# FFmpeg/FFmpeg

Hardware: AMD Instinct MI355X
Metric: swscale_nv12_1080p_to_4k_bicubic_Mpixels_per_s (higher is better)
Workload: dtype u8

## Files before the change

### ffmpeg_amd/csrc/kernels/sws_kernels.h

```cpp
#ifndef FFHIP_SWS_KERNELS_H
#define FFHIP_SWS_KERNELS_H

#include <hip/hip_runtime.h>
#include <stddef.h>
#include <stdint.h>

__host__ __device__ __forceinline__ uint32_t sws_block_numbering(uint32_t b, uint32_t nb, int mode)
{
    if (mode == 1) {
        const uint32_t x = b & 7u, sl = b >> 3, q = nb >> 3, r = nb & 7u;
        return (x < r ? x * (q + 1u) : r * (q + 1u) + (x - r) * q) + sl;
    }
    if (mode > 1) {
        const uint32_t lg = (uint32_t)mode - 1u, C = 1u << lg, full = nb & ~(8u * C - 1u);
        if (b < full) {
            const uint32_t x = b & 7u, sl = b >> 3;
            return (((sl >> lg) << 3) + x) * C + (sl & (C - 1u));
        }
    }
    return b;
}

struct FFHipYuv2RgbK {
    int cy;
// ... 27 lines not shown

struct FFHipDevFilter {
    const int16_t *filter;
    const int32_t *pos;
    int size, n;
};

struct FFHipScalePlaneArgs {
    const uint8_t *src[2];
    uint8_t *dst[2];
    ptrdiff_t src_stride[2], dst_stride[2];
    size_t src_fp[2], dst_fp[2];
    int src_step, dst_step;
    int srcW, srcH, dstW, dstH;
    int nframes;
    FFHipDevFilter h, v;
    int tw, th;
    int max_cols, max_rows;
    int tiles_x, tiles_y;
    int rc_coeff, rc_offset, rc_clip;
};
int ffhip_launch_scale_yuv(const FFHipScalePlaneArgs &lum, const FFHipScalePlaneArgs &chr, hipStream_t stream);
int ffhip_plan_scale_plane(FFHipScalePlaneArgs *a, int channels, const int32_t *hpos_host, const int32_t *vpos_host);


struct FFHipCwJob {
    const uint8_t *src[2];
    uint8_t *dst[2];
    ptrdiff_t sstride[2], dstride[2];
    size_t sfp[2], dfp[2];
    int kind, src_swap, dst_swap;
    int srcW, srcH, dstW, dstH;
    const int16_t *hf; const int32_t *hp;
    const int16_t *vf; const int32_t *vp;
    int ncb, nstrips, strip_rows, unit_begin;
};
struct FFHipCwArgs {
    FFHipCwJob job[3];
    int njobs, units_per_frame, nframes, flags;
};
int  ffhip_cw_bank_nowrap(const int16_t *filter, int size, int n);
int  ffhip_cw_bank_dup12(const int32_t *hpos, int hn);
int  ffhip_cw_bank_ok(const int32_t *hpos, int hsize, int hn, int srcW, const int32_t *vpos, int vsize, int vn, int srcH);
void ffhip_cw_plan_job(FFHipCwJob *j, int groups_per_lane, int strip_target);
int  ffhip_launch_colwalk(FFHipCwArgs &A, int luma_groups, int depth, hipStream_t stream);

struct FFHipUp2Job {
    const uint8_t *src; uint8_t *dst;
    ptrdiff_t sstride, dstride;
    size_t sfp, dfp;
    int pair, swap;
    int srcW, srcH;
    int ngroups;
    const uint32_t *hfv;
    const uint32_t *vfv;
    int nfull, upj;
    int nstrips, steps_per_strip, unit_begin;
    int hb_sdepth, hb_ddepth, hb_smsb, hb_dmsb;
    int rc_coeff, rc_offset;
    uint32_t hco[16];
    int hco_ok;
};
struct FFHipUp2Args {
    FFHipUp2Job job[3];
    int njobs, units_per_pack, npacks, nframes, fshift;
    int xcd;
};
#ifdef __cplusplus
#include <vector>
int  ffhip_up2_virtual_bank(const int16_t *filter, const int32_t *pos, int n_dst, int n_src, std::vector<uint32_t> *out);
int  ffhip_up2_hco(const std::vector<uint32_t> &h, uint32_t out[16]);
#endif
void ffhip_up2_plan_job(FFHipUp2Job *j, int lanes_per_frame, int want_steps);
int  ffhip_launch_up2(FFHipUp2Args &A, int depth, int var, hipStream_t stream);

struct FFHipUp2RgbArgs {
    const uint8_t *src[3];
    uint8_t *dst;
    ptrdiff_t sstride[3], dstride;
    size_t sfp[3], dfp;
    int sil, swap;
    int srcW, srcH;
    int ngroups;
    int nframes;
    const uint32_t *hco;
    const uint32_t *vt;
    int nstrips, steps_per_strip;
    int fpp, wpp, npacks;
    int vround;
    int lay;
    FFHipYuv2RgbK k;
};
#ifdef __cplusplus
int  ffhip_upn_virtual_bank(const int16_t *filter, const int32_t *pos, int n_dst, int n_src, int ratio, std::vector<uint32_t> *out);
int  ffhip_up2rgb_hco(const std::vector<uint32_t> &hl, const std::vector<uint32_t> &hc, uint32_t out[32]);
#endif
void ffhip_up2rgb_plan(FFHipUp2RgbArgs *a, int want_steps, int fpp_forced);
int  ffhip_launch_up2rgb(FFHipUp2RgbArgs &A, int var, hipStream_t stream);

struct FFHipDn2Job {
    const uint8_t *src; uint8_t *dst;
    ptrdiff_t sstride, dstride;
    size_t sfp, dfp;
    int pair, swap;
    int srcH, dstH;
    int ngroups;
// ... 303 lines not shown
```

### ffmpeg_amd/csrc/kernels/sws_up2.hip

```cpp
#include <stdlib.h>
#include <type_traits>
#include <vector>

#include "common.h"
#include "sws_kernels.h"

typedef uint32_t up_u2 __attribute__((ext_vector_type(2)));
typedef uint32_t up_u3 __attribute__((ext_vector_type(3)));
typedef uint32_t up_u4 __attribute__((ext_vector_type(4)));
typedef uint32_t up_u8 __attribute__((ext_vector_type(8)));
typedef up_u3 __attribute__((aligned(4))) up_u3a;
typedef const uint8_t __attribute__((address_space(1))) *up_gcp;
typedef uint8_t __attribute__((address_space(1))) *up_gp;
typedef const up_u3a __attribute__((address_space(1))) *up_gc3;
typedef up_u2 __attribute__((address_space(1))) *up_g2;
typedef up_u4 __attribute__((aligned(4))) up_u4a;
typedef up_u2 __attribute__((aligned(4))) up_u2a;
typedef const up_u4a __attribute__((address_space(1))) *up_gc4;
typedef const up_u2a __attribute__((address_space(1))) *up_gc2;
typedef up_u4a __attribute__((address_space(1))) *up_g4;
typedef const up_u8 __attribute__((address_space(4))) *up_cc8;

struct UpRaw { uint32_t q[3]; };
struct UpRawH { uint32_t q[6]; };
// ... 96 lines not shown

__device__ __forceinline__ void up_v8h(uint32_t (&w)[4], const uint32_t (&pa)[8], const uint32_t (&pb)[8], uint32_t f01, uint32_t f23,
                                       int kround, int sh, uint32_t maxpk)
{
    int t0, t1, t2, t3, t4, t5, t6, t7;
    asm("v_dot2_i32_i16 %4, %12, %28, %30\n\t"
        "v_dot2_i32_i16 %5, %13, %28, %30\n\t"
        "v_dot2_i32_i16 %6, %14, %28, %30\n\t"
        "v_dot2_i32_i16 %7, %15, %28, %30\n\t"
        "v_dot2_i32_i16 %8, %16, %28, %30\n\t"
        "v_dot2_i32_i16 %9, %17, %28, %30\n\t"
        "v_dot2_i32_i16 %10, %18, %28, %30\n\t"
        "v_dot2_i32_i16 %11, %19, %28, %30\n\t"
        "v_dot2_i32_i16 %4, %20, %29, %4\n\t"
        "v_dot2_i32_i16 %5, %21, %29, %5\n\t"
        "v_dot2_i32_i16 %6, %22, %29, %6\n\t"
        "v_dot2_i32_i16 %7, %23, %29, %7\n\t"
        "v_dot2_i32_i16 %8, %24, %29, %8\n\t"
        "v_dot2_i32_i16 %9, %25, %29, %9\n\t"
        "v_dot2_i32_i16 %10, %26, %29, %10\n\t"
        "v_dot2_i32_i16 %11, %27, %29, %11\n\t"
        "v_ashrrev_i32 %4, %31, %4\n\t"
        "v_ashrrev_i32 %5, %31, %5\n\t"
        "v_ashrrev_i32 %6, %31, %6\n\t"
        "v_ashrrev_i32 %7, %31, %7\n\t"
        "v_ashrrev_i32 %8, %31, %8\n\t"
        "v_ashrrev_i32 %9, %31, %9\n\t"
        "v_ashrrev_i32 %10, %31, %10\n\t"
        "v_ashrrev_i32 %11, %31, %11\n\t"
        "v_cvt_pk_i16_i32 %0, %4, %5\n\t"
        "v_cvt_pk_i16_i32 %1, %6, %7\n\t"
        "v_cvt_pk_i16_i32 %2, %8, %9\n\t"
        "v_cvt_pk_i16_i32 %3, %10, %11\n\t"
        "v_pk_max_i16 %0, %0, 0\n\t"
        "v_pk_max_i16 %1, %1, 0\n\t"
        "v_pk_max_i16 %2, %2, 0\n\t"
        "v_pk_max_i16 %3, %3, 0\n\t"
        "v_pk_min_i16 %0, %0, %32\n\t"
        "v_pk_min_i16 %1, %1, %32\n\t"
        "v_pk_min_i16 %2, %2, %32\n\t"
        "v_pk_min_i16 %3, %3, %32"
        : "=&v"(w[0]), "=&v"(w[1]), "=&v"(w[2]), "=&v"(w[3]), "=&v"(t0), "=&v"(t1), "=&v"(t2), "=&v"(t3), "=&v"(t4), "=&v"(t5), "=&v"(t6),
          "=&v"(t7)
        : "v"(pa[0]), "v"(pa[1]), "v"(pa[2]), "v"(pa[3]), "v"(pa[4]), "v"(pa[5]), "v"(pa[6]), "v"(pa[7]),
          "v"(pb[0]), "v"(pb[1]), "v"(pb[2]), "v"(pb[3]), "v"(pb[4]), "v"(pb[5]), "v"(pb[6]), "v"(pb[7]),
          "s"(f01), "s"(f23), "v"(kround), "v"(sh), "v"(maxpk));
}

template <int PAIR, int D, int VAR, int HB = 0, int RC = 0, int SC = 0>
__device__ __forceinline__ void up2_unit(const FFHipUp2Job &J, int frame0, int fshift, int gbase, int strip, int lane, int nframes)
{
    constexpr bool DBG_NOST = VAR & 16, DBG_ROW0 = VAR & 32, DBG_COPY = VAR & 64;
    constexpr bool NTS = VAR & 1;
    const int lpf = 64 >> fshift;
    const int fsub = lane >> (6 - fshift);
    const int gl = lane & (lpf - 1);
    const int graw = gbase + gl, fraw = frame0 + fsub;
    const bool act = graw < J.ngroups && fraw < nframes;
    const int g = min(graw, J.ngroups - 1);
    const int fs = fraw < nframes ? fsub : 0;
    const bool lb = g == 0, rb = g == J.ngroups - 1;
    const bool border = gbase == 0 || gbase + lpf >= J.ngroups;

    const uint32_t soff = (uint32_t)fs * (uint32_t)J.sfp +
                          (uint32_t)(!HB ? (lb ? 0 : rb ? 4 * g - 8 : 4 * g - 4)
                                     : PAIR ? (lb ? 0 : rb ? 8 * g - 16 : 8 * g - 8) : (lb ? 0 : rb ? 8 * g - 8 : 8 * g - 4));
    const uint32_t doff = (uint32_t)fs * (uint32_t)J.dfp + (HB ? 16u : 8u) * (uint32_t)g;
    const int hsh = HB ? J.hb_sdepth - 1 : 7, vsh = HB ? 27 - J.hb_ddepth : 19;
    const uint32_t maxpk = HB ? ((1u << J.hb_ddepth) - 1) * 0x00010001u : 0;
    const int smsb = HB ? (J.hb_smsb ? 16 - J.hb_sdepth : 0) : 0, dmsb = HB ? (J.hb_dmsb ? 16 - J.hb_ddepth : 0) : 0;

    constexpr int NCF = SC ? 4 : PAIR ? 8 : 16;
    uint32_t cf[NCF];
    if (!SC) {
        const up_u4 *p = reinterpret_cast<const up_u4 *>(J.hfv) + (size_t)g * (NCF / 4);
#pragma unroll
        for (int i = 0; i < NCF / 4; i++) {
            const up_u4 v = p[i];
            cf[4 * i] = v.x; cf[4 * i + 1] = v.y; cf[4 * i + 2] = v.z; cf[4 * i + 3] = v.w;
        }
    }
    const uint32_t cE0 = J.hco[0], cE1 = J.hco[1], cO0 = J.hco[2], cO1 = J.hco[3];
    const uint32_t par = PAIR ? (J.swap ? 0x00010001u : 0u) : 0u;
    const uint32_t sA0 = 0x0c020c00u + par, sA1 = 0x0c040c02u + par, sA2 = 0x0c060c04u + par;
    const uint32_t sB0 = 0x0c030c01u - par, sB1 = 0x0c050c03u - par, sB2 = 0x0c070c05u - par;
    const uint32_t fixl = PAIR ? 0x01000100u : 0x00000000u, fixr = PAIR ? 0x03020302u : 0x03030303u;

    const int S = J.steps_per_strip;
    const int a = 1 + strip * S, b = min(a + S, J.srcH + 2);
    const uint8_t *sbase = J.src + (size_t)frame0 * J.sfp;
    uint8_t *dbase = J.dst + (size_t)frame0 * J.dfp;
    const ptrdiff_t sstride = J.sstride, dstride = J.dstride;
    const int srcH = J.srcH, dstH = 2 * J.srcH;
    int pr = a - 3;
    const uint8_t *pf = sbase + (ptrdiff_t)min(max(pr, 0), srcH - 1) * sstride;
    uint8_t *dr = dbase + (ptrdiff_t)(2 * a - 3) * dstride;
    asm("" : "+s"(pf), "+s"(dr));

    typedef typename std::conditional<HB != 0, UpRawH, UpRaw>::type Raw;
    auto load_next = [&](Raw &o) {
        uint32_t off = soff;
        asm volatile("" : "+v"(off));
        if (HB) {
            const up_u4 w = *(up_gc4)((up_gcp)pf + off);
            o.q[0] = w.x; o.q[1] = w.y; o.q[2] = w.z; o.q[3] = w.w;
            if (PAIR) {
                const up_u2 x = *(up_gc2)((up_gcp)pf + off + 16);
                o.q[4] = x.x; o.q[5] = x.y;
            }
        } else {
            const up_u3 w = *(up_gc3)((up_gcp)pf + off);
            o.q[0] = w.x; o.q[1] = w.y; o.q[2] = w.z;
        }
        pr++;
        if (!DBG_ROW0)
            pf += (pr >= 1 && pr <= srcH - 1) ? sstride : 0;
        asm("" : "+s"(pf));
    };

    uint32_t ring[3][8];
    int hprev[8];
#pragma unroll
    for (int i = 0; i < 8; i++)
        hprev[i] = 0;
    int kround = HB ? 1 << (vsh - 1) : 64 << 12;
    asm volatile("" : "+v"(kround));

    auto hpass = [&](const Raw &w, uint32_t (&Pnew)[8]) {
        int h[8];
        if (HB) {
            uint32_t v[6];
            constexpr int NQ = PAIR ? 6 : 4;
#pragma unroll
            for (int i = 0; i < NQ; i++)
                v[i] = w.q[i];
            if (border) {
                if (PAIR) {
                    const uint32_t q0 = w.q[0], q1 = w.q[1], q2 = w.q[2], q3 = w.q[3], q4 = w.q[4], q5 = w.q[5];
                    v[0] = lb ? q0 : rb ? q2 : q0; v[1] = lb ? q0 : rb ? q3 : q1; v[2] = lb ? q0 : rb ? q4 : q2;
                    v[3] = lb ? q1 : rb ? q5 : q3; v[4] = lb ? q2 : rb ? q5 : q4; v[5] = lb ? q3 : rb ? q5 : q5;
                } else {
                    const uint32_t q0 = w.q[0], q1 = w.q[1], q2 = w.q[2], q3 = w.q[3];
                    const uint32_t f0 = __builtin_amdgcn_perm(q0, q0, 0x01000100u), f3 = __builtin_amdgcn_perm(q3, q3, 0x03020302u);
                    v[0] = lb ? f0 : rb ? q1 : q0; v[1] = lb ? q0 : rb ? q2 : q1;
                    v[2] = lb ? q1 : rb ? q3 : q2; v[3] = lb ? q2 : rb ? f3 : q3;
                }
            }
            if (smsb) {
                typedef unsigned short up_h2 __attribute__((ext_vector_type(2)));
#pragma unroll
                for (int i = 0; i < NQ; i++)
                    v[i] = __builtin_bit_cast(uint32_t, __builtin_bit_cast(up_h2, v[i]) >> (unsigned short)smsb);
            }
            if (PAIR) {
                uint32_t a[5], b[5];
#pragma unroll
                for (int k = 0; k < 5; k++) {
                    a[k] = __builtin_amdgcn_perm(v[k + 1], v[k], 0x05040100u);
                    b[k] = __builtin_amdgcn_perm(v[k + 1], v[k], 0x07060302u);
                }
                int ha[4], hb[4];
                up_h4s(ha, a[0], a[1], a[1], a[2], a[2], a[3], a[3], a[4], cf, hsh);
                up_h4s(hb, b[0], b[1], b[1], b[2], b[2], b[3], b[3], b[4], cf, hsh);
#pragma unroll
                for (int i = 0; i < 4; i++) {
                    h[2 * i] = ha[i];
                    h[2 * i + 1] = hb[i];
                }
            } else {
                const uint32_t p0 = v[0], p2 = v[1], p4 = v[2], p6 = v[3];
                const uint32_t p1 = __builtin_amdgcn_alignbyte(v[1], v[0], 2), p3 = __builtin_amdgcn_alignbyte(v[2], v[1], 2);
                const uint32_t p5 = __builtin_amdgcn_alignbyte(v[3], v[2], 2);
                int hl[4], hh[4];
                up_h4s(hl, p0, p1, p1, p2, p2, p3, p3, p4, cf, hsh);
                up_h4s(hh, p2, p3, p3, p4, p4, p5, p5, p6, cf + 8, hsh);
#pragma unroll
                for (int i = 0; i < 4; i++) {
                    h[i] = hl[i];
                    h[4 + i] = hh[i];
                }
            }
#pragma unroll
            for (int i = 0; i < 8; i++) {
// ... 232 lines not shown
    return 1;
}

int ffhip_up2_hco(const std::vector<uint32_t> &v, uint32_t out[16])
{
    const int n = (int)(v.size() / 2);
    if (n < 16 || (n & 1))
        return 0;
    for (int x = 3; x < n - 3; x++)
        if (v[2 * (size_t)x] != v[2 * (size_t)(4 + (x & 1))] || v[2 * (size_t)x + 1] != v[2 * (size_t)(4 + (x & 1)) + 1])
            return 0;
    for (int i = 0; i < 4; i++)
        out[i] = v[8 + i];
    for (int i = 0; i < 6; i++) {
        out[4 + i] = v[i];
        out[10 + i] = v[2 * (size_t)(n - 3) + i];
    }
    return 1;
}

void ffhip_up2_plan_job(FFHipUp2Job *j, int lanes_per_frame, int want)
{
    const int steps = j->srcH + 1;
    int n = cdiv(steps, want);
    int s = cdiv(cdiv(steps, n), 6) * 6;
    j->steps_per_strip = s;
    j->nstrips = cdiv(steps, s);
    if (lanes_per_frame == 64) {
        j->nfull = 0;
        j->upj = cdiv(j->ngroups, 64);
    } else {
        j->nfull = j->ngroups / 64;
        j->upj = j->nfull * (64 / lanes_per_frame) + cdiv(j->ngroups - j->nfull * 64, lanes_per_frame);
    }
}

int ffhip_launch_up2(FFHipUp2Args &A, int depth, int var, hipStream_t stream)
{
    if (A.nframes <= 0)
        return 0;
    int u = 0;
    for (int i = 0; i < A.njobs; i++) {
        A.job[i].unit_begin = u;
        u += A.job[i].upj * A.job[i].nstrips;
    }
    A.units_per_pack = u;
    A.npacks = (A.nframes + (1 << A.fshift) - 1) >> A.fshift;
    const long long waves = (long long)u * A.npacks;
    if (waves >= (1LL << 31)) {
        ffhip_set_error("ffhip_sws: batch too large for one launch (%lld waves)", waves);
        return FFHIP_EINVAL;
    }
    const dim3 grid((unsigned)((waves + 3) / 4)), block(256);
    if (A.job[0].hb_sdepth) {
        if (depth == 3 && !(var & 1))      hipLaunchKernelGGL((k_sws_up2<3, 0, 1>), grid, block, 0, stream, A);
        else if (depth == 3)               hipLaunchKernelGGL((k_sws_up2<3, 1, 1>), grid, block, 0, stream, A);
        else if (!(var & 1))               hipLaunchKernelGGL((k_sws_up2<6, 0, 1>), grid, block, 0, stream, A);
        else                               hipLaunchKernelGGL((k_sws_up2<6, 1, 1>), grid, block, 0, stream, A);
        LAUNCH_CHECK();
        return 0;
    }
    if (A.job[0].rc_coeff) {
        bool scr = var == 3;
        for (int i = 0; i < A.njobs; i++)
            scr = scr && A.job[i].hco_ok;
        if (scr && depth == 3)             hipLaunchKernelGGL((k_sws_up2<3, 1, 0, 1, 1>), grid, block, 0, stream, A);
        else if (scr)                      hipLaunchKernelGGL((k_sws_up2<6, 1, 0, 1, 1>), grid, block, 0, stream, A);
        else if (depth == 3)               hipLaunchKernelGGL((k_sws_up2<3, 0, 0, 1>), grid, block, 0, stream, A);
        else                               hipLaunchKernelGGL((k_sws_up2<6, 0, 0, 1>), grid, block, 0, stream, A);
        LAUNCH_CHECK();
        return 0;
    }
    bool sc = true;
    for (int i = 0; i < A.njobs; i++)
        sc = sc && A.job[i].hco_ok;
    if (var == 2 || var == 3) {
        if (!sc)
            var &= 1;
        else {
            if (var == 2 && depth == 3) hipLaunchKernelGGL((k_sws_up2<3, 0, 0, 0, 1>), grid, block, 0, stream, A);
            else if (var == 2)          hipLaunchKernelGGL((k_sws_up2<6, 0, 0, 0, 1>), grid, block, 0, stream, A);
            else if (depth == 3)        hipLaunchKernelGGL((k_sws_up2<3, 1, 0, 0, 1>), grid, block, 0, stream, A);
            else                        hipLaunchKernelGGL((k_sws_up2<6, 1, 0, 0, 1>), grid, block, 0, stream, A);
            LAUNCH_CHECK();
            return 0;
        }
    }
#define UP2_LAUNCH(DD, VV) hipLaunchKernelGGL((k_sws_up2<DD, VV>), grid, block, 0, stream, A)
#define UP2_CASE(VV) case VV: if (depth == 3) UP2_LAUNCH(3, VV); else UP2_LAUNCH(6, VV); break
    switch (var) {
    UP2_CASE(0);
    UP2_CASE(1);
    UP2_CASE(16); UP2_CASE(48); UP2_CASE(64);
    default:
        ffhip_set_error("ffhip_sws: exact-2x kernel variant %d is not built", var);
        return FFHIP_EINVAL;
    }
#undef UP2_CASE
#undef UP2_LAUNCH
    LAUNCH_CHECK();
    return 0;
}
```

### ffmpeg_amd/csrc/sws_api.hip

```cpp
#include <initializer_list>
#include <mutex>
#include <new>
#include <stdlib.h>
#include <string.h>
#include <utility>
#include <vector>

#include "kernels/common.h"
#include "kernels/sws_kernels.h"
#include "kernels/shim_arena.h"

struct DevBlock {
    void *p = nullptr;
    DevBlock() = default;
    DevBlock(const DevBlock &) = delete;
    DevBlock &operator=(const DevBlock &) = delete;
    DevBlock(DevBlock &&o) noexcept : p(o.p) { o.p = nullptr; }
    DevBlock &operator=(DevBlock &&o) noexcept { std::swap(p, o.p); return *this; }
    ~DevBlock() { if (p) (void)hipFree(p); }
};

static hipError_t grow(DevBlock &b, size_t &sz, size_t need)
{
    if (need <= sz)
// ... 53 lines not shown
        d[i].pos = static_cast<const int32_t *>(at[2 * i + 1]);
    }
    return true;
}

struct Scratch {
    DevBlock buf;
    size_t sz = 0;
    std::mutex mu;
    hipEvent_t done = nullptr;
    ~Scratch() { if (done) (void)hipEventDestroy(done); }
};
struct ScratchLease {
    Scratch *s = nullptr;
    hipStream_t stream = nullptr;
    std::unique_lock<std::mutex> lk;
    ~ScratchLease() { if (s) (void)hipEventRecord(s->done, stream); }
};
static hipError_t acquire(Scratch &s, ScratchLease &l, size_t need, hipStream_t stream)
{
    l.lk = std::unique_lock<std::mutex>(s.mu);
    hipError_t e = s.done ? hipStreamWaitEvent(stream, s.done, 0) : hipEventCreateWithFlags(&s.done, hipEventDisableTiming);
    if (e == hipSuccess)
        e = grow(s.buf, s.sz, need);
    if (e == hipSuccess) {
        l.s = &s;
        l.stream = stream;
    }
    return e;
}

struct FFHipSwsRgbIn {
    int bpp = 0;
    int half = 0;
    int direct_c = 0;
    int fused420 = 0;
    DevBlock vfv;
    int y_direct = 0;
    int fmt = 0;
    int ofs[3] = { 0, 0, 0 };
    int32_t table[9] = {};
    DevBlock stage;
    size_t stage_sz = 0;
};
static void rgb_in_plan_luma(struct FFHipSwsContext *c);
static thread_local int g_sws_create_flat_dither = 0;

struct FFHipSwsContext {
    int device = 0;
    FFHipSwsRgbIn rgb_in;
    int hrgb_seed0 = 0;
    int widen8 = 0;
    Scratch widen_tmp;
    Scratch rgb_in_planes;
    bool rgb_in_luma_done = false;
    int flat_dither = 0;
    int hbd_sw = 320, hbd_rows = 96;
    int hbd = 0;
    FFHipSwsTables t;
    std::vector<int16_t> f[4];
    std::vector<int32_t> p[4];
    DevBlock dev_tables;
    FFHipDevFilter d[4];
    int unscaled_yuv2rgb = 0;
    FFHipYuv2RgbK k;
    int chrSrcW, chrSrcH;
    FFHipScalePlaneArgs lum, chr;
    FFHipScaleRgbArgs rgb;
    std::vector<int16_t> nf[4];
    std::vector<int32_t> np[4];
    DevBlock dev_ntables;
    FFHipDevFilter dn[4];
    int cw_ok = 0;
    int cw_opt = 0;
    int cw_dup = 0;
    int cw_rgb = 0;
    int cw_vround = 1 << 18;
    int lw_ok = 0, lw_ht = 0, lw_vt = 0;
    std::vector<int16_t> wf[4];
    std::vector<int32_t> wp[4];
    DevBlock dev_wtables;
    FFHipDevFilter dw[4];
    int w16_ok = 0, w16_ht = 0, w16_vt = 0;
    DevBlock w16_dev;
    int w16_span[2][3] = {};
    FFHipDevFilter w16[4] = {};
    int up2_ok = 0;
    int up2_rc = 0;
    DevBlock up2_dev;
    const uint32_t *up2_h[2] = { nullptr, nullptr }, *up2_v[2] = { nullptr, nullptr };
    hipEvent_t tune_ev[16] = {};
    int tune_n = 0, tune_choice = -1;
    uint32_t up2_hco[2][16] = {};
    int up2_hco_ok[2] = { 0, 0 };
    int eqr_ok = 0;
    DevBlock eqr_dev;
    Scratch rgb2_tmp;
    hipStream_t rgb2_aux = nullptr;
    hipEvent_t rgb2_fork = nullptr, rgb2_join = nullptr;
    int u2r_ok = 0;
    DevBlock u2r_dev;
    const uint32_t *u2r_hco = nullptr, *u2r_vt = nullptr;
    int dn2_ok = 0;
    int mix_up2 = 0;
    int mix_dn2 = 0;
    int c420_ok = 0;
// ... 475 lines not shown
        }
        if (hrgb && (t->full_chr_h_int || (t->dstW & 1) || t->dst_alpha_fill == 2 || c->flat_dither)) {
            ffhip_set_error("ffhip_sws: above 8 bits into packed RGB: full-chroma writers (odd width / 4:4:4 source / SWS_FULL_CHR_H_INT) and alpha are not on the hip path");
            ffhip_sws_freeContext(c);
            return nullptr;
        }
        if (c->d[1].n != (hrgb ? (t->dstW + 1) >> 1 : -((-t->dstW) >> fmt_hsub(t->dstFormat))) ||
            c->d[3].n != (hrgb ? t->dstH : -((-t->dstH) >> fmt_vsub(t->dstFormat))) ||
            c->d[0].n != t->dstW || c->d[2].n != t->dstH) {
            ffhip_set_error("ffhip_sws: the banks do not match the target's plane sizes");
            ffhip_sws_freeContext(c);
            return nullptr;
        }
        c->hbd = 2;
        c->hbd_sw = 8;
        c->hbd_rows = 1;
        for (int b = 0; b < 2; b++) {
            const std::vector<int32_t> &pos = c->p[b];
            const int fs = c->d[b].size, n = c->d[b].n;
            for (int x0 = 0; x0 < n; x0 += 64) {
                const int x1 = (x0 + 63 < n ? x0 + 63 : n - 1);
                int lo = pos[x0], hi = pos[x0];
                for (int x = x0; x <= x1; x++) { lo = pos[x] < lo ? pos[x] : lo; hi = pos[x] > hi ? pos[x] : hi; }
                if (hi + fs - lo > 320 || lo != pos[x0])
                    c->hbd = 1;
                else if (hi + fs - lo > c->hbd_sw)
                    c->hbd_sw = hi + fs - lo;
            }
            const std::vector<int32_t> &vp = c->p[2 + b];
            const int vfs = c->d[2 + b].size, vn = c->d[2 + b].n;
            for (int y0 = 0; y0 < vn; y0 += 32) {
                const int y1 = (y0 + 31 < vn ? y0 + 31 : vn - 1);
                if (vp[y1] + vfs - vp[y0] > c->hbd_rows)
                    c->hbd_rows = vp[y1] + vfs - vp[y0];
            }
        }
        c->hbd_sw = (c->hbd_sw + 3) & ~1;
        {
            int sd = 8, sl = 0, dd = 8, dl = 0;
            (void)ffhip_pixfmt_hbd(t->srcFormat, &sd, &sl, nullptr, nullptr);
            (void)ffhip_pixfmt_hbd(t->dstFormat, &dd, &dl, nullptr, nullptr);
            const int cw = c->chrSrcW, chh = c->chrSrcH;
            const bool nowrap = bank_nowrap_depth(c->f[0].data(), c->d[0].n, sd, c->d[0].size) && bank_nowrap_depth(c->f[1].data(), c->d[1].n, sd, c->d[1].size);
            const int limits[4] = { t->srcW, cw, t->srcH, chh };
            const bool w8 = sd == 8 && dd > 8 && dd <= 14 && !c->flat_dither && t->srcFormat != FFHIP_PIX_FMT_NV21 &&
                            (fmt_nv(t->srcFormat) ? dl == 1 : dl == 0);
            if (((sd > 8 && sd <= 14 && sl == dl && sl != 2) || w8) && dd > 8 && dd <= 14 && t->src_range == t->dst_range &&
                t->dstW == 2 * t->srcW && t->dstH == 2 * t->srcH && c->d[1].n == 2 * cw && c->d[3].n == 2 * chh &&
                !(t->srcW & 3) && t->srcW >= 8 && (sl ? !(cw & 1) && cw >= 4 : !(cw & 3) && cw >= 8) &&
                build_fast_view(c, limits, false) && bank_nowrap_depth(c->nf[0].data(), c->d[0].n, sd) &&
                bank_nowrap_depth(c->nf[1].data(), c->d[1].n, sd)) {
                up2_build(c, limits);
                c->widen8 = c->up2_ok && w8;
            }
            const int cdw = c->d[1].n, cdh = c->d[3].n;
            const bool dn8 = dd == 8 && !hrgb && !c->flat_dither  && (sl == 1 ? t->dstFormat == FFHIP_PIX_FMT_NV12 : !fmt_nv(t->dstFormat));
            if (sd > 8 && sd <= 14 && ((dd > 8 && dd <= 14 && sl == dl) || dn8) && sl != 2 && t->src_range == t->dst_range &&
                t->srcW == 2 * t->dstW && t->srcH == 2 * t->dstH && cw == 2 * cdw && chh == 2 * cdh &&
                !(t->dstW & 3) && t->dstW >= 12 && (sl ? !(cdw & 1) && cdw >= 6 : !(cdw & 3) && cdw >= 12) && nowrap)
                dn2_build(c, limits);
            {
                const bool w8u = sd == 8 && dd > 8 && dd <= 14 && !c->flat_dither && t->srcFormat != FFHIP_PIX_FMT_NV21 &&
                                 (fmt_nv(t->srcFormat) ? dl == 1 : dl == 0);
                if (((sd > 8 && sd <= 14 && sl == dl && sl != 2) || w8u) && dd > 8 && dd <= 14 && !hrgb && !c->flat_dither && t->src_range == t->dst_range &&
                    2 * t->dstW == 3 * t->srcW && 2 * t->dstH == 3 * t->srcH && 2 * c->d[1].n == 3 * cw && 2 * c->d[3].n == 3 * chh &&
                    !(t->srcW & 3) && t->srcW >= 12 && !(t->srcH & 1) && !(chh & 1) &&
                    ((sl || fmt_nv(t->srcFormat)) ? !(cw & 1) && cw >= 6 : !(cw & 3) && cw >= 12) && nowrap)
                    u32_build(c, limits, 2, 3);
                if (((sd > 8 && sd <= 14 && sl == dl && sl != 2) || w8u) && dd > 8 && dd <= 14 && !hrgb && !c->flat_dither && t->src_range == t->dst_range &&
                    3 * t->dstW == 4 * t->srcW && 3 * t->dstH == 4 * t->srcH && 3 * c->d[1].n == 4 * cw && 3 * c->d[3].n == 4 * chh &&
                    !(t->srcW % 6) && t->srcW >= 18 && !(t->srcH % 3) && !(chh % 3) &&
                    ((sl || fmt_nv(t->srcFormat)) ? !(cw % 3) && cw >= 9 : !(cw % 6) && cw >= 18) && nowrap)
                    u32_build(c, limits, 3, 4);
                if (c->u32_ok && w8u)
                    c->widen8 = 1;
            }
            if (sd > 8 && sd <= 14 && ((dd > 8 && dd <= 14 && sl == dl) || dn8) && sl != 2 && !hrgb && !c->flat_dither && t->src_range == t->dst_range &&
                2 * t->srcW == 3 * t->dstW && 2 * t->srcH == 3 * t->dstH && 2 * cw == 3 * cdw && 2 * chh == 3 * cdh &&
                !(t->dstW & 3) && t->dstW >= 12 && !(t->dstH & 1) && !(cdh & 1) && (sl ? !(cdw & 1) && cdw >= 6 : !(cdw & 3) && cdw >= 12) && nowrap)
                d32_build(c, limits);
            if (!c->d32_ok && sd > 8 && sd <= 14 && dd > 8 && dd <= 14 && sl == dl && sl != 2 && !hrgb && !c->flat_dither && t->src_range == t->dst_range &&
                3 * t->srcW == 4 * t->dstW && 3 * t->srcH == 4 * t->dstH && 3 * cw == 4 * cdw && 3 * chh == 4 * cdh &&
                !(t->dstW % 6) && t->dstW >= 18 && !(t->dstH % 3) && !(cdh % 3) && (sl ? !(cdw % 3) && cdw >= 9 : !(cdw % 6) && cdw >= 18) && nowrap)
                d32_build(c, limits, 4, 3);
            const bool to8 = dd == 8 && (t->dstFormat == FFHIP_PIX_FMT_NV12 || !fmt_nv(t->dstFormat));
            const bool widen = sd == 8 && dd > 8 && dd <= 14 && t->srcFormat != FFHIP_PIX_FMT_NV21 && !c->flat_dither;
            if (!c->up2_ok && !c->dn2_ok && ((sd > 8 && sd <= 14) || widen) && ((dd > 8 && dd <= 14) || to8) && (sl != 2 || widen) && dl != 2 &&
                (t->src_range == t->dst_range || hrgb ) &&
                c->d[0].size <= 16 && c->d[1].size <= 16 && c->d[2].size <= 16 && c->d[3].size <= 16 && nowrap) {
                const int hmax = c->d[0].size > c->d[1].size ? c->d[0].size : c->d[1].size, vmax = c->d[2].size > c->d[3].size ? c->d[2].size : c->d[3].size;
                int ht = hmax <= 4 ? 4 : hmax <= 8 ? 8 : 16, vt = vmax <= 4 ? 4 : vmax <= 8 ? 8 : 16;
                if (ht == 16 && vt == 4) vt = 8;
                if (vt == 16 && ht == 4) ht = 8;
                const int T[4] = { ht, ht, vt, vt };
                std::vector<int16_t> pf[4];
                std::vector<int32_t> pp[4];
                bool ok = true;
                for (int i = 0; i < 4 && ok; i++)
                    ok = ffhip_w16_pad_bank(c->f[i].data(), c->p[i].data(), c->d[i].size, c->d[i].n, limits[i], T[i], &pf[i], &pp[i]);
                if (ok && upload_banks(c->w16_dev, pf, pp, 256, c->w16)) {
                    c->w16_ht = ht;
                    c->w16_vt = vt;
                    c->w16_ok = 1;
                    c->widen8 = widen;
                    for (int i = 0; i < 2; i++) {
                        c->w16_span[i][0] = ffhip_w16_span(pp[i].data(), c->d[i].n, 256, 2, ht);
// ... 310 lines not shown
        vb.resize((size_t)(c->d[3].n + 8) * 4, 0);
        void *at[1];
        c->rgb_in.fused420 = upload(c->rgb_in.vfv, { part(vb) }, 4, at);
    }
}

static FFHipRgbInArgs rgb_in_args(const FFHipSwsContext *c, const void *src, ptrdiff_t src_stride, size_t src_fp, int rows)
{
    FFHipRgbInArgs a;
    memset(&a, 0, sizeof(a));
    a.src = static_cast<const uint8_t *>(src); a.src_stride = src_stride; a.src_fp = src_fp;
    a.w = c->t.srcW; a.h = rows;
    a.ro = c->rgb_in.ofs[0]; a.go = c->rgb_in.ofs[1]; a.bo = c->rgb_in.ofs[2];
    const int32_t *T = c->rgb_in.table;
    a.ry = T[0]; a.gy = T[1]; a.by = T[2]; a.ru = T[3]; a.gu = T[4]; a.bu = T[5]; a.rv = T[6]; a.gv = T[7]; a.bv = T[8];
    return a;
}

static int rgb_in_launch(const FFHipSwsContext *c, int nframes, const uint8_t *src, ptrdiff_t src_stride, size_t src_fp, int rows, uint8_t *const p[3],
                         const int pitch[3], const size_t fp[3], hipStream_t stream, uint8_t *y8 = nullptr, ptrdiff_t y8_stride = 0, size_t y8_fp = 0)
{
    FFHipRgbInArgs a = rgb_in_args(c, src, src_stride, src_fp, rows);
    a.y8 = y8; a.y8_stride = y8_stride; a.y8_fp = y8_fp;
    for (int i = 0; i < 3; i++) {
        a.dst[i] = p[i]; a.dst_stride[i] = pitch[i]; a.dst_fp[i] = fp[i];
    }
    return ffhip_launch_sws_rgb_in(a, c->rgb_in.bpp, c->rgb_in.half, nframes, stream);
}

extern "C" int ffhip_sws_set_yuv2rgb(FFHipSwsContext *c, const FFHipSwsTables *t)
{
    if (!c || !t)
        return FFHIP_EINVAL;
    std::lock_guard<std::mutex> lk(c->mu);
    FFHipSwsTables n = c->t;
    n.yuv2rgb_cy = t->yuv2rgb_cy; n.yuv2rgb_oy = t->yuv2rgb_oy; n.yuv2rgb_crv = t->yuv2rgb_crv; n.yuv2rgb_cbu = t->yuv2rgb_cbu;
    n.yuv2rgb_cgu = t->yuv2rgb_cgu; n.yuv2rgb_cgv = t->yuv2rgb_cgv; n.yuv2rgb_yoffs = t->yuv2rgb_yoffs;
    for (int i = 0; i < 6; i++)
        n.yuv2rgb_full[i] = t->yuv2rgb_full[i];
    FFHipYuv2RgbK k;
    const int r = make_k(n, &k);
    if (r < 0)
        return r;
    c->t = n;
    c->k = k;
    c->rgb.k = k;
    for (int i = 0; i < 6; i++)
        c->rgb.fk[i] = n.yuv2rgb_full[i];
    return 0;
}

extern "C" int ffhip_sws_fast_path(const FFHipSwsContext *c)
{
    return c ? (c->cw_ok || c->cw_rgb) + (c->mf_ok ? 2 : 0) + (c->lw_ok ? 4 : 0) + (c->up2_ok ? 8 : 0) + (c->dn2_ok ? 16 : 0) + (c->w16_ok ? 32 : 0) + (c->u2r_ok ? 64 : 0) + (c->eqr_ok ? 128 : 0) + (c->f444_ok ? 256 : 0) + (c->c420_ok ? 512 : 0) + (c->mix_dn2 ? 1024 : 0) + (c->mix_up2 ? 2048 : 0) + (c->d32_ok ? 4096 : 0) + (c->u32_ok ? 8192 : 0) : 0;
}

extern "C" int ffhip_sws_tuned_numbering(const FFHipSwsContext *c)
{
    return c ? c->tune_choice : -1;
}

extern "C" int ffhip_sws_mfma_tiles_host(const int16_t *filter, const int32_t *pos, int n, int srcW, int pair, int src_swap,
                                         uint8_t *out, size_t out_size)
{
    std::vector<uint8_t> v;
    const int nt = ffhip_mf_build_tiles(&v, filter, pos, n, srcW, pair, src_swap);
    if (nt < 0)
        return FFHIP_EINVAL;
    if (out) {
        if (out_size < v.size())
            return FFHIP_ENOMEM;
        memcpy(out, v.data(), v.size());
    }
    return nt;
}

extern "C" int ffhip_sws_up2_virtual_bank_host(const int16_t *filter, const int32_t *pos, int n_dst, int n_src, uint32_t *out)
{
    std::vector<uint32_t> v;
    if (!filter || !pos || !out || !ffhip_up2_virtual_bank(filter, pos, n_dst, n_src, &v))
        return 0;
    memcpy(out, v.data(), v.size() * 4);
    return 1;
}

extern "C" int ffhip_sws_upn_virtual_bank_host(const int16_t *filter, const int32_t *pos, int n_dst, int n_src, int ratio, uint32_t *out)
{
    std::vector<uint32_t> v;
    if (!filter || !pos || !out || !ffhip_upn_virtual_bank(filter, pos, n_dst, n_src, ratio, &v))
        return 0;
    memcpy(out, v.data(), v.size() * 4);
    return 1;
}

extern "C" int ffhip_sws_up2rgb_hco_host(const uint32_t *hl, int n_hl, const uint32_t *hc, int n_hc, uint32_t out[32])
{
    if (!hl || !hc || !out || n_hl <= 0 || n_hc <= 0)
        return 0;
    const std::vector<uint32_t> a(hl, hl + (size_t)n_hl * 2), b(hc, hc + (size_t)n_hc * 2);
    return ffhip_up2rgb_hco(a, b, out);
}

extern "C" int ffhip_sws_down2_virtual_bank_host(const int16_t *filter, const int32_t *pos, int fsize, int n_dst, int n_src, uint32_t *out)
{
    std::vector<uint32_t> v;
    if (!filter || !pos || !out || !ffhip_down2_virtual_bank(filter, pos, fsize, n_dst, n_src, &v))
        return 0;
// ... 89 lines not shown

template <class A> static void put_src(A &a, const SidePlanes &s)
{
    for (int i = 0; i < 3; i++) {
        a.src[i] = i && s.il ? s.pair : s.p[i];
        a.sstride[i] = s.stride[i];
        a.sfp[i] = s.fp[i];
    }
}

static int up2_fshift(const FFHipUp2Args &U, int nframes)
{
    int best = -1;
    double bestw = 1e30;
    for (int fsft = 0; fsft <= 2; fsft++) {
        const int lpf = 64 >> fsft;
        bool fits = !(nframes < (1 << fsft) && fsft);
        double w = 0;
        for (int i = 0; i < U.njobs; i++) {
            const FFHipUp2Job &j = U.job[i];
            const unsigned long long span_s = (unsigned long long)((1 << fsft) - 1) * j.sfp + (unsigned long long)j.srcH * (size_t)(j.sstride < 0 ? -j.sstride : j.sstride);
            const unsigned long long span_d = (unsigned long long)((1 << fsft) - 1) * j.dfp + 2ull * j.srcH * (size_t)(j.dstride < 0 ? -j.dstride : j.dstride);
            if (span_s >= (1ull << 31) || span_d >= (1ull << 31))
                fits = false;
            const int nfull = fsft ? j.ngroups / 64 : 0;
            w += ((double)nfull + (double)cdiv(j.ngroups - nfull * 64, lpf) / (1 << fsft)) * j.srcH;
        }
        if (fits && w < bestw - 1e-9) {
            bestw = w;
            best = fsft;
        }
    }
    return best;
}

static int scale16(FFHipSwsContext *c, int nframes, const void *const src[4], const int srcStride[4], const size_t srcFramePitch[4],
                   void *const dst[4], const int dstStride[4], const size_t dstFramePitch[4], hipStream_t stream)
{
    const FFHipSwsTables &t = c->t;
    int sd = 8, sl = fmt_nv(t.srcFormat) ? 2 : 0, dd = 8, dl = fmt_nv(t.dstFormat) ? 2 : 0;
    (void)ffhip_pixfmt_hbd(t.srcFormat, &sd, &sl, nullptr, nullptr);
    (void)ffhip_pixfmt_hbd(t.dstFormat, &dd, &dl, nullptr, nullptr);
    const int ssz = sd > 8 ? 2 : 1, dsz = dd > 8 ? 2 : 1;
    const bool hrgb = fmt_rgb(t.dstFormat);
    for (int pl = 0; pl < (sl ? 2 : 3); pl++)
        if (!src[pl] || (srcStride[pl] % ssz) || (srcFramePitch[pl] % ssz) || ((uintptr_t)src[pl] % ssz))
            return FFHIP_EINVAL;
    for (int pl = 0; pl < (hrgb ? 1 : dl ? 2 : 3); pl++)
        if (!dst[pl] || (dstStride[pl] % dsz) || (dstFramePitch[pl] % dsz) || ((uintptr_t)dst[pl] % dsz))
            return FFHIP_EINVAL;
    const SidePlanes cs = side_planes(src, srcStride, srcFramePitch, sl ? 2 : 3, false, ssz);
    const SidePlanes d = side_planes(dst, dstStride, dstFramePitch, hrgb ? 1 : dl ? 2 : 3, false, dsz);
    SidePlanes ws = cs;
    ScratchLease wlease;
    bool widened = false;
    if (c->widen8 && (c->w16_ok || c->up2_ok || c->u32_ok) && d.pos && !(d.al() & 3) && cs.pos &&
        !knob_is(c->up2_ok ? "FFHIP_SWS_UP2" : "FFHIP_SWS_WALK16", '0')) {
        const int np = sl ? 2 : 3;
        const int wb[3] = { t.srcW, sl ? 2 * c->chrSrcW : c->chrSrcW, c->chrSrcW }, rows[3] = { t.srcH, c->chrSrcH, c->chrSrcH };
        size_t pitch[3], fp[3], off[3], need = 0;
        for (int pl = 0; pl < np; pl++) {
            pitch[pl] = ((size_t)2 * wb[pl] + 255) & ~(size_t)255;
            fp[pl] = pitch[pl] * (size_t)rows[pl];
            off[pl] = need;
            need += fp[pl] * (size_t)nframes;
        }
        HIP_TRY(acquire(c->widen_tmp, wlease, need, stream));
        const void *wsrc[4] = {};
        int wss[4] = {};
        size_t wsf[4] = {};
        for (int pl = 0; pl < np; pl++) {
            uint8_t *w = static_cast<uint8_t *>(c->widen_tmp.buf.p) + off[pl];
            const int r = ffhip_launch_sws_widen8(static_cast<const uint8_t *>(src[pl]), srcStride[pl], srcFramePitch[pl], w, (ptrdiff_t)pitch[pl], fp[pl],
                                                  wb[pl], rows[pl], nframes, stream);
            if (r < 0)
                return r;
            wsrc[pl] = w; wss[pl] = (int)pitch[pl]; wsf[pl] = fp[pl];
        }
        widened = true;
        sl = sl ? 1 : 0;
        ws = side_planes(wsrc, wss, wsf, np, false, 2);
    }
    const uintptr_t al = ws.al() | (hrgb ? 0 : d.al());
    const bool neg = ws.neg || d.neg;
    const int sw[2] = { t.srcW, c->chrSrcW }, sh[2] = { t.srcH, c->chrSrcH };
    if (c->up2_ok && (widened || !c->widen8) && !(al & 3) && !neg && !knob_is("FFHIP_SWS_UP2", '0')) {
        FFHipUp2Args U;
        memset(&U, 0, sizeof(U));
        U.nframes = nframes;
        U.xcd = 1;
        for_each_job(ws, d, true, true, [&](const PlaneJob &q) {
            FFHipUp2Job &j = U.job[U.njobs++];
            put_planes(j, q);
            j.swap = q.swap;
            j.srcW = sw[q.which]; j.srcH = sh[q.which];
            j.ngroups = q.pair ? j.srcW / 2 : j.srcW / 4;
            j.hfv = c->up2_h[q.which]; j.vfv = c->up2_v[q.which];
            j.hb_sdepth = sd; j.hb_ddepth = dd; j.hb_smsb = sl == 1 && !widened; j.hb_dmsb = dl == 1;
        });
        const int fs = up2_fshift(U, nframes);
        if (fs >= 0) {
            U.fshift = fs;
            for (int i = 0; i < U.njobs; i++)
                ffhip_up2_plan_job(&U.job[i], 64 >> U.fshift, 60);
            const char *ev2 = FFHIP_KNOB("FFHIP_UP2_VAR");
            return ffhip_launch_up2(U, knob_is("FFHIP_UP2_DEPTH", '3') ? 3 : 6, ev2 ? atoi(ev2) : 0, stream);
        }
    }
    if (c->dn2_ok && !(al & 3) && !neg && !knob_is("FFHIP_SWS_DOWN2", '0')) {
        FFHipDn2Args D;
        memset(&D, 0, sizeof(D));
        D.nframes = nframes;
        D.xcd = 1;
        for_each_job(cs, d, true, true, [&](const PlaneJob &q) {
            FFHipDn2Job &j = D.job[D.njobs++];
            put_planes(j, q);
            j.swap = q.swap;
            j.srcH = sh[q.which]; j.dstH = c->d[2 + q.which].n;
            j.ngroups = q.pair ? c->d[q.which].n / 2 : c->d[q.which].n / 4;
            j.hfv = c->dn2_h[q.which]; j.vfv = c->dn2_v[q.which];
            j.hb_sdepth = sd; j.hb_ddepth = dd; j.hb_smsb = sl == 1; j.hb_dmsb = dd > 8 && dl == 1;
            j.dither_off = q.plane == 2 ? 3 : 0;
            ffhip_down2_plan_job(&j, 32);
        });
        return ffhip_launch_down2(D, stream);
    }
    if (hrgb && !(c->w16_ok && !(al & 3) && !neg)) {
        ffhip_set_error("ffhip_sws: above 8 bits into packed RGB needs 4-byte aligned planes and pitches, top-down");
        return FFHIP_EINVAL;
    }
    if (c->d32_ok && !hrgb && !widened && !c->widen8 && !(al & 3) && !neg && !knob_is("FFHIP_SWS_DOWN32", '0')) {
        FFHipD32Args D;
        memset(&D, 0, sizeof(D));
        D.nframes = nframes;
        D.hb = 1; D.sdepth = sd; D.ddepth = dd; D.smsb = sl == 1; D.dmsb = dl == 1;
        D.ratio43 = c->d32_ok == 2;
        const int pin = D.ratio43 ? 4 : 3, pout = D.ratio43 ? 3 : 2;
        for_each_job(cs, d, true, true, [&](const PlaneJob &q) {
            FFHipD32Job &j = D.job[D.njobs++];
            put_planes(j, q);
            j.swap = q.swap;
            j.srcH = sh[q.which]; j.dstH = j.srcH / pin * pout;
            j.ngroups = q.pair ? c->d[q.which].n / pout : c->d[q.which].n / (2 * pout);
            j.hfv = c->d32_h[q.which]; j.vfv = c->d32_v[q.which];
            j.dither_off = q.plane == 2 ? 3 : 0;
        });
        return ffhip_launch_down32(D, stream);
    }
    if (c->u32_ok && !hrgb && (widened || !c->widen8) && !(al & 3) && !neg && !knob_is("FFHIP_SWS_UP32", '0')) {
        FFHipU32Args U;
        memset(&U, 0, sizeof(U));
        U.nframes = nframes;
        U.sdepth = sd; U.ddepth = dd; U.smsb = sl == 1 && !widened; U.dmsb = dl == 1;
        U.ratio43 = c->u32_ok == 2;
        const int pin = U.ratio43 ? 3 : 2, pout = U.ratio43 ? 4 : 3;
        for_each_job(ws, d, true, true, [&](const PlaneJob &q) {
            FFHipU32Job &j = U.job[U.njobs++];
            put_planes(j, q);
            j.srcH = sh[q.which]; j.dstH = j.srcH / pin * pout;
            j.ngroups = q.pair ? c->d[q.which].n / pout : c->d[q.which].n / (2 * pout);
// ... 1210 lines not shown
```

Before: 2.804 million.

## Read 8-bit sources directly in up2 kernel, skipping the widen8 pre-pass

Adds an HB=2 template mode to the 2x upscale kernel that loads 8-bit source rows directly while keeping the high-bit-depth output path. The host then launches this mode before the separate widen8 kernel, which used to copy the planes into a 16-bit scratch buffer. This drops one kernel launch and a full read-write pass over the source through scratch memory. In exchange it adds template variants and new eligibility checks on width and alignment.

Measured after the change: 2.793 million, median of 2. Within noise of the previous version (-0.4%).

```diff
diff --git a/ffmpeg_amd/csrc/kernels/sws_kernels.h b/ffmpeg_amd/csrc/kernels/sws_kernels.h
--- a/ffmpeg_amd/csrc/kernels/sws_kernels.h
+++ b/ffmpeg_amd/csrc/kernels/sws_kernels.h
@@ -103,6 +103,7 @@
     int pair, swap;
     int srcW, srcH;
     int ngroups;
+    int src8;
     const uint32_t *hfv;
     const uint32_t *vfv;
     int nfull, upj;
diff --git a/ffmpeg_amd/csrc/kernels/sws_up2.hip b/ffmpeg_amd/csrc/kernels/sws_up2.hip
--- a/ffmpeg_amd/csrc/kernels/sws_up2.hip
+++ b/ffmpeg_amd/csrc/kernels/sws_up2.hip
@@ -172,6 +172,7 @@
 {
     constexpr bool DBG_NOST = VAR & 16, DBG_ROW0 = VAR & 32, DBG_COPY = VAR & 64;
     constexpr bool NTS = VAR & 1;
+    constexpr bool SH = HB == 1;
     const int lpf = 64 >> fshift;
     const int fsub = lane >> (6 - fshift);
     const int gl = lane & (lpf - 1);
@@ -183,12 +184,12 @@
     const bool border = gbase == 0 || gbase + lpf >= J.ngroups;
 
     const uint32_t soff = (uint32_t)fs * (uint32_t)J.sfp +
-                          (uint32_t)(!HB ? (lb ? 0 : rb ? 4 * g - 8 : 4 * g - 4)
+                          (uint32_t)(!SH ? (lb ? 0 : rb ? 4 * g - 8 : 4 * g - 4)
                                      : PAIR ? (lb ? 0 : rb ? 8 * g - 16 : 8 * g - 8) : (lb ? 0 : rb ? 8 * g - 8 : 8 * g - 4));
     const uint32_t doff = (uint32_t)fs * (uint32_t)J.dfp + (HB ? 16u : 8u) * (uint32_t)g;
-    const int hsh = HB ? J.hb_sdepth - 1 : 7, vsh = HB ? 27 - J.hb_ddepth : 19;
+    const int hsh = SH ? J.hb_sdepth - 1 : 7, vsh = HB ? 27 - J.hb_ddepth : 19;
     const uint32_t maxpk = HB ? ((1u << J.hb_ddepth) - 1) * 0x00010001u : 0;
-    const int smsb = HB ? (J.hb_smsb ? 16 - J.hb_sdepth : 0) : 0, dmsb = HB ? (J.hb_dmsb ? 16 - J.hb_ddepth : 0) : 0;
+    const int smsb = SH ? (J.hb_smsb ? 16 - J.hb_sdepth : 0) : 0, dmsb = HB ? (J.hb_dmsb ? 16 - J.hb_ddepth : 0) : 0;
 
     constexpr int NCF = SC ? 4 : PAIR ? 8 : 16;
     uint32_t cf[NCF];
@@ -217,11 +218,11 @@
     uint8_t *dr = dbase + (ptrdiff_t)(2 * a - 3) * dstride;
     asm("" : "+s"(pf), "+s"(dr));
 
-    typedef typename std::conditional<HB != 0, UpRawH, UpRaw>::type Raw;
+    typedef typename std::conditional<SH, UpRawH, UpRaw>::type Raw;
     auto load_next = [&](Raw &o) {
         uint32_t off = soff;
         asm volatile("" : "+v"(off));
-        if (HB) {
+        if (SH) {
             const up_u4 w = *(up_gc4)((up_gcp)pf + off);
             o.q[0] = w.x; o.q[1] = w.y; o.q[2] = w.z; o.q[3] = w.w;
             if (PAIR) {
@@ -248,7 +249,7 @@
 
     auto hpass = [&](const Raw &w, uint32_t (&Pnew)[8]) {
         int h[8];
-        if (HB) {
+        if (SH) {
             uint32_t v[6];
             constexpr int NQ = PAIR ? 6 : 4;
 #pragma unroll
@@ -587,6 +588,20 @@
         return FFHIP_EINVAL;
     }
     const dim3 grid((unsigned)((waves + 3) / 4)), block(256);
+    if (A.job[0].src8) {
+        bool sc8 = !(var & 4);
+        for (int i = 0; i < A.njobs; i++)
+            sc8 = sc8 && A.job[i].hco_ok;
+#define UP2_SRC8(DD, VV) do { if (sc8) hipLaunchKernelGGL((k_sws_up2<DD, VV, 2, 0, 1>), grid, block, 0, stream, A); \
+                              else     hipLaunchKernelGGL((k_sws_up2<DD, VV, 2, 0, 0>), grid, block, 0, stream, A); } while (0)
+        if (depth == 3 && !(var & 1))      UP2_SRC8(3, 0);
+        else if (depth == 3)               UP2_SRC8(3, 1);
+        else if (!(var & 1))               UP2_SRC8(6, 0);
+        else                               UP2_SRC8(6, 1);
+#undef UP2_SRC8
+        LAUNCH_CHECK();
+        return 0;
+    }
     if (A.job[0].hb_sdepth) {
         if (depth == 3 && !(var & 1))      hipLaunchKernelGGL((k_sws_up2<3, 0, 1>), grid, block, 0, stream, A);
         else if (depth == 3)               hipLaunchKernelGGL((k_sws_up2<3, 1, 1>), grid, block, 0, stream, A);
diff --git a/ffmpeg_amd/csrc/sws_api.hip b/ffmpeg_amd/csrc/sws_api.hip
--- a/ffmpeg_amd/csrc/sws_api.hip
+++ b/ffmpeg_amd/csrc/sws_api.hip
@@ -129,6 +129,7 @@
     int hrgb_seed0 = 0;
     int widen8 = 0;
     Scratch widen_tmp;
+    int up2_src8 = 0;
     Scratch rgb_in_planes;
     bool rgb_in_luma_done = false;
     int flat_dither = 0;
@@ -710,6 +711,7 @@
                 bank_nowrap_depth(c->nf[1].data(), c->d[1].n, sd)) {
                 up2_build(c, limits);
                 c->widen8 = c->up2_ok && w8;
+                c->up2_src8 = c->widen8 && t->srcW >= 12 && (fmt_nv(t->srcFormat) ? cw >= 6 : cw >= 12);
             }
             const int cdw = c->d[1].n, cdh = c->d[3].n;
             const bool dn8 = dd == 8 && !hrgb && !c->flat_dither  && (sl == 1 ? t->dstFormat == FFHIP_PIX_FMT_NV12 : !fmt_nv(t->dstFormat));
@@ -1126,7 +1128,7 @@
 
 extern "C" int ffhip_sws_fast_path(const FFHipSwsContext *c)
 {
-    return c ? (c->cw_ok || c->cw_rgb) + (c->mf_ok ? 2 : 0) + (c->lw_ok ? 4 : 0) + (c->up2_ok ? 8 : 0) + (c->dn2_ok ? 16 : 0) + (c->w16_ok ? 32 : 0) + (c->u2r_ok ? 64 : 0) + (c->eqr_ok ? 128 : 0) + (c->f444_ok ? 256 : 0) + (c->c420_ok ? 512 : 0) + (c->mix_dn2 ? 1024 : 0) + (c->mix_up2 ? 2048 : 0) + (c->d32_ok ? 4096 : 0) + (c->u32_ok ? 8192 : 0) : 0;
+    return c ? (c->cw_ok || c->cw_rgb) + (c->mf_ok ? 2 : 0) + (c->lw_ok ? 4 : 0) + (c->up2_ok ? 8 : 0) + (c->dn2_ok ? 16 : 0) + (c->w16_ok ? 32 : 0) + (c->u2r_ok ? 64 : 0) + (c->eqr_ok ? 128 : 0) + (c->f444_ok ? 256 : 0) + (c->c420_ok ? 512 : 0) + (c->mix_dn2 ? 1024 : 0) + (c->mix_up2 ? 2048 : 0) + (c->d32_ok ? 4096 : 0) + (c->u32_ok ? 8192 : 0) + (c->up2_src8 ? 16384 : 0) : 0;
 }
 
 extern "C" int ffhip_sws_tuned_numbering(const FFHipSwsContext *c)
@@ -1322,6 +1324,41 @@
     const SidePlanes cs = side_planes(src, srcStride, srcFramePitch, sl ? 2 : 3, false, ssz);
     const SidePlanes d = side_planes(dst, dstStride, dstFramePitch, hrgb ? 1 : dl ? 2 : 3, false, dsz);
     SidePlanes ws = cs;
+    const int sw[2] = { t.srcW, c->chrSrcW }, sh[2] = { t.srcH, c->chrSrcH };
+    auto up2_launch = [&](const SidePlanes &s, bool widened, bool bytes, int *ret) {
+        FFHipUp2Args U;
+        memset(&U, 0, sizeof(U));
+        U.nframes = nframes;
+        U.xcd = 1;
+        for_each_job(s, d, true, true, [&](const PlaneJob &q) {
+            FFHipUp2Job &j = U.job[U.njobs++];
+            put_planes(j, q);
+            j.swap = q.swap;
+            j.srcW = sw[q.which]; j.srcH = sh[q.which];
+            j.ngroups = q.pair ? j.srcW / 2 : j.srcW / 4;
+            j.hfv = c->up2_h[q.which]; j.vfv = c->up2_v[q.which];
+            j.hb_sdepth = sd; j.hb_ddepth = dd; j.hb_smsb = sl == 1 && !widened && !bytes; j.hb_dmsb = dl == 1;
+            if (bytes) {
+                j.src8 = 1;
+                j.hco_ok = c->up2_hco_ok[q.which];
+                memcpy(j.hco, c->up2_hco[q.which], sizeof(j.hco));
+            }
+        });
+        const int fs = up2_fshift(U, nframes);
+        if (fs < 0)
+            return 0;
+        U.fshift = fs;
+        for (int i = 0; i < U.njobs; i++)
+            ffhip_up2_plan_job(&U.job[i], 64 >> U.fshift, 60);
+        const char *ev2 = FFHIP_KNOB("FFHIP_UP2_VAR");
+        *ret = ffhip_launch_up2(U, knob_is("FFHIP_UP2_DEPTH", '3') ? 3 : 6, ev2 ? atoi(ev2) : 0, stream);
+        return 1;
+    };
+    if (c->up2_src8 && d.pos && cs.pos && !((d.al() | cs.al()) & 3) && !knob_is("FFHIP_SWS_UP2", '0') && !knob_is("FFHIP_UP2_SRC8", '0')) {
+        int r = 0;
+        if (up2_launch(cs, false, true, &r))
+            return r;
+    }
     ScratchLease wlease;
     bool widened = false;
     if (c->widen8 && (c->w16_ok || c->up2_ok || c->u32_ok) && d.pos && !(d.al() & 3) && cs.pos &&
@@ -1353,29 +1390,10 @@
     }
     const uintptr_t al = ws.al() | (hrgb ? 0 : d.al());
     const bool neg = ws.neg || d.neg;
-    const int sw[2] = { t.srcW, c->chrSrcW }, sh[2] = { t.srcH, c->chrSrcH };
     if (c->up2_ok && (widened || !c->widen8) && !(al & 3) && !neg && !knob_is("FFHIP_SWS_UP2", '0')) {
-        FFHipUp2Args U;
-        memset(&U, 0, sizeof(U));
-        U.nframes = nframes;
-        U.xcd = 1;
-        for_each_job(ws, d, true, true, [&](const PlaneJob &q) {
-            FFHipUp2Job &j = U.job[U.njobs++];
-            put_planes(j, q);
-            j.swap = q.swap;
-            j.srcW = sw[q.which]; j.srcH = sh[q.which];
-            j.ngroups = q.pair ? j.srcW / 2 : j.srcW / 4;
-            j.hfv = c->up2_h[q.which]; j.vfv = c->up2_v[q.which];
-            j.hb_sdepth = sd; j.hb_ddepth = dd; j.hb_smsb = sl == 1 && !widened; j.hb_dmsb = dl == 1;
-        });
-        const int fs = up2_fshift(U, nframes);
-        if (fs >= 0) {
-            U.fshift = fs;
-            for (int i = 0; i < U.njobs; i++)
-                ffhip_up2_plan_job(&U.job[i], 64 >> U.fshift, 60);
-            const char *ev2 = FFHIP_KNOB("FFHIP_UP2_VAR");
-            return ffhip_launch_up2(U, knob_is("FFHIP_UP2_DEPTH", '3') ? 3 : 6, ev2 ? atoi(ev2) : 0, stream);
-        }
+        int r = 0;
+        if (up2_launch(ws, widened, false, &r))
+            return r;
     }
     if (c->dn2_ok && !(al & 3) && !neg && !knob_is("FFHIP_SWS_DOWN2", '0')) {
         FFHipDn2Args D;
```
